# VIDILabs/open-volume-renderer

Hardware: AMD Instinct MI355X
Metric: Msamples/s (primary ray-march samples after ERT); fps alongside (higher is better)
Workload: dtype f32

## Files before the change

### open-volume-renderer_amd/csrc/ovr_hip_kernels.hip

```cpp
#include "ovr_hip_device.h"

namespace ovrhip {
static_assert(kPoolSubs <= 64 && (kPoolSubs & (kPoolSubs - 1)) == 0, "reduce_counters_kernel reduces the sub-pool counters with one wave");
__global__ __launch_bounds__(kBlock) void composite_kernel(const RayMarchParams P)
{
  const int lane = threadIdx.x & 63, wave = threadIdx.x >> 6;
  int ix, iy;
  const bool active = assign_pixel_quad(P, lane, wave, ix, iy) && (lane & 3) == 0;
  const PoolDesc& Q = P.pool;
  if (Q.ctrl[1] != 0u) return;
  const unsigned int tile = blockIdx.x * kWaves + wave;
  const unsigned int pixel_index = (unsigned int)ix + (unsigned int)iy * (unsigned int)P.width;
  float alpha = 0.f;
  unsigned int first = 0;
  int pend = 0;
  if (active) {
    const float4 st = Q.pix_state[pixel_index];
    alpha = st.x; first = __float_as_uint(st.y); pend = __float_as_int(st.z);
  }
  f3 color = mk3(0, 0, 0), gradient = mk3(0, 0, 0);
  const unsigned int total = Q.tile_count[tile];
  auto load_chunk = [&](int c, unsigned int n) {
    ShadeReq r;
    r.px = r.py = r.pz = r.s = r.v = r.tr = r.a = 0.f; r.next = 0;
    if ((unsigned int)lane < n) r = Q.reqs[(size_t)c * 64 + lane];
    return r;
  };
  int c = total > 0u ? Q.tile_first[tile] : 0;
  int link = total > 0u ? Q.chunk_next[c | (kRun - 1)] : 0;
  ShadeReq r = load_chunk(c, min(total, 64u));
  for (unsigned int base = 0; base < total; base += 64u) {
    const unsigned int n = min(total - base, 64u);
    const bool more = base + 64u < total;
    const bool run_end = (c & (kRun - 1)) == kRun - 1;
    const int c_next = run_end ? link : c + 1;
    ShadeReq r_next = r;
    if (more) {
      r_next = load_chunk(c_next, min(total - base - 64u, 64u));
      if (run_end) link = Q.chunk_next[c_next | (kRun - 1)];
    }
    apply_batch(r, base, n, lane, pend, first, color, gradient);
    r = r_next;
    c = c_next;
  }
  if (active) {
    f3 o_c = mk3(0, 0, 0), o_g = mk3(0, 0, 0);
    if (alpha > 0.f) {
      o_c = mk3(color.x / alpha, color.y / alpha, color.z / alpha);
      o_g = mk3(gradient.x / alpha, gradient.y / alpha, gradient.z / alpha);
    }
    float o_a = alpha;
    if (P.spp > 1) {
      float4* sr = reinterpret_cast<float4*>(P.spp_sum_rgba) + pixel_index;
      float* sg = P.spp_sum_grad + 3ull * pixel_index;
      float4 acc = make_float4(0.f, 0.f, 0.f, 0.f);
      f3 accg = mk3(0, 0, 0);
      if (P.spp_index > 0) { acc = *sr; accg = mk3(sg[0], sg[1], sg[2]); }
      acc.x += o_c.x; acc.y += o_c.y; acc.z += o_c.z; acc.w += alpha;
      accg.x += o_g.x; accg.y += o_g.y; accg.z += o_g.z;
      if (P.spp_index + 1 < P.spp) {
        *sr = acc; sg[0] = accg.x; sg[1] = accg.y; sg[2] = accg.z;
        return;
      }
      if (Q.ctrl[32 * (kPoolSubs + 1)] > Q.sub_capacity) return;
      const float rspp = 1.f / (float)P.spp;
      o_a = acc.w * rspp;
      o_c = mk3(acc.x * rspp, acc.y * rspp, acc.z * rspp);
      o_g = mk3(accg.x * rspp, accg.y * rspp, accg.z * rspp);
    }
    write_pixel(P, pixel_index, o_c, o_a, o_g);
  }
}

__global__ __launch_bounds__(256) void reduce_counters_kernel(const unsigned int* __restrict__ partials, int n_blocks, const unsigned int* __restrict__ shade_partials,
                                                             int n_shade_blocks, unsigned long long* counters, unsigned int* pool_ctrl,
                                                             unsigned long long* publish, unsigned int* done, unsigned int* conv_asked)
{
  if (pool_ctrl && blockIdx.x == 0 && threadIdx.x < 64) {
    unsigned int v = threadIdx.x < (unsigned int)kPoolSubs ? pool_ctrl[32u * (threadIdx.x + 1u)] : 0u;
#pragma unroll
    for (int off = 32; off > 0; off >>= 1) v = max(v, (unsigned int)__shfl_xor((int)v, off));
    if (threadIdx.x == 0) atomicMax(&pool_ctrl[32 * (kPoolSubs + 1)], v);
  }
  __shared__ unsigned long long red[4][kNC];
  unsigned long long acc[kNC] = {};
  const int stride = gridDim.x * 256;
  for (int b = blockIdx.x * 256 + threadIdx.x; b < n_blocks; b += stride) {
#pragma unroll
    for (int c = 0; c < kNC; ++c) acc[c] += partials[(size_t)b * kNC + c];
  }
  if (shade_partials)
    for (int b = blockIdx.x * 256 + threadIdx.x; b < n_shade_blocks; b += stride) {
      acc[3] += shade_partials[2 * b];
      acc[6] += shade_partials[2 * b + 1];
    }
#pragma unroll
  for (int c = 0; c < kNC; ++c) {
    for (int off = 32; off > 0; off >>= 1) acc[c] += __shfl_down(acc[c], off);
  }
  const int lane = threadIdx.x & 63, wave = threadIdx.x >> 6;
  if (lane == 0) {
#pragma unroll
    for (int c = 0; c < kNC; ++c) red[wave][c] = acc[c];
  }
  __syncthreads();
  if (threadIdx.x < kNC) atomicAdd(&counters[threadIdx.x], red[0][threadIdx.x] + red[1][threadIdx.x] + red[2][threadIdx.x] + red[3][threadIdx.x]);
  if (!publish) return;
  __shared__ unsigned int ticket;
  __threadfence();
  __syncthreads();
  if (threadIdx.x == 0) ticket = atomicAdd(done, 1u);
  __syncthreads();
  if (ticket != gridDim.x - 1u) return;
  __threadfence();
  if (threadIdx.x < 8) {
    publish[threadIdx.x] = threadIdx.x < kNC ? __hip_atomic_load(&counters[threadIdx.x], __ATOMIC_RELAXED, __HIP_MEMORY_SCOPE_AGENT) : 0ull;
    counters[threadIdx.x] = 0ull;
  }
  unsigned int* pub_ctrl = reinterpret_cast<unsigned int*>(publish + 8);
  if (pool_ctrl)
    for (int i = threadIdx.x; i < kPoolCtrlWords; i += 256) {
      const unsigned int w = __hip_atomic_load(&pool_ctrl[i], __ATOMIC_RELAXED, __HIP_MEMORY_SCOPE_AGENT);
      pub_ctrl[i] = w;
      pool_ctrl[i] = 0u;
      if (conv_asked && i == 32 * (kPoolSubs + 1)) *conv_asked = w;
    }
  else if (conv_asked && threadIdx.x == 0) *conv_asked = 0u;
  if (threadIdx.x == 0) *done = 0u;
}
constexpr int kSchedClasses = 64;
__device__ __forceinline__ float schedule_probe(const RayMarchParams& P, const MarchConsts& mc, unsigned int e, int k)
{
  const f3 c0 = ld3(P.cam_dir), h0 = ld3(P.cam_hor), v0 = ld3(P.cam_ver);
  const f3 oo = to_object(mc, ld3(P.cam_pos));
  const int bx = (int)(e & 0xffffu) * 8, by = (int)(e >> 16) * 8;
  const int ix = min(bx + (k == 0 ? 4 : (k & 1) ? 0 : 7), P.width - 1), iy = min(by + (k == 0 ? 4 : (k & 2) ? 0 : 7), P.height - 1);
  const float ux = ((float)ix + .5f) / (float)P.width - 0.5f, uy = ((float)iy + .5f) / (float)P.height - 0.5f;
  const f3 d = normalize3_exact(mk3(c0.x + ux * h0.x + uy * v0.x, c0.y + ux * h0.y + uy * v0.y, c0.z + ux * h0.z + uy * v0.z));
  float a = 0.f, b = FLT_MAX;
  if (intersect_unit_box(a, b, oo, mk3(d.x * mc.inv_scale.x, d.y * mc.inv_scale.y, d.z * mc.inv_scale.z))) return b - a;
  return -1.f;
}
__device__ __forceinline__ unsigned int schedule_class_of(const RayMarchParams& P, float longest)
{
  if (!(longest >= 0.f)) return 0u;
  const float rel = longest / (P.long_ray_steps * P.step);
  return (unsigned int)min(kSchedClasses - 1, 1 + (int)(rel * (float)(kSchedClasses - 2)));
}

__global__ __launch_bounds__(256) void schedule_classify_kernel(const RayMarchParams P, const unsigned int* __restrict__ src, unsigned int n, int exact,
                                                               unsigned int* __restrict__ cls)
{
  VolConsts vc;
  MarchConsts mc;
  setup_consts(P, vc, mc);
  const unsigned int i = blockIdx.x * 4u + (threadIdx.x >> 6);
  if (i >= n) return;
  const int lane = threadIdx.x & 63;
  const unsigned int e = src[i];
  const int ix = (int)(e & 0xffffu) * 8 + (lane & 7), iy = (int)(e >> 16) * 8 + (lane >> 3);
  bool active = ix < P.width && iy < P.height;
  if (P.world > 1 && active) active = ((ix / P.tile_w + iy / P.tile_h) % P.world) == P.rank;
  const bool hit = exact == 1 && active && pixel_ray_hits_box(P, mc, ix, iy);
  const unsigned long long any = __ballot(hit), act = __ballot(active);
  bool culled = false;
  if (exact == 2) {
    const float x0 = ((float)((int)(e & 0xffffu) * 8) - 1.5f) / (float)P.width - 0.5f, x1 = ((float)((int)(e & 0xffffu) * 8 + 8) + 1.5f) / (float)P.width - 0.5f;
    const float y0 = ((float)((int)(e >> 16) * 8) - 1.5f) / (float)P.height - 0.5f, y1 = ((float)((int)(e >> 16) * 8 + 8) + 1.5f) / (float)P.height - 0.5f;
    const f3 cd = ld3(P.cam_dir), ch = ld3(P.cam_hor), cv = ld3(P.cam_ver);
    auto ray = [&](int k) {
      const float ux = (k == 1 || k == 2) ? x1 : x0, uy = (k >= 2) ? y1 : y0;
      return mk3((cd.x + ux * ch.x + uy * cv.x) * mc.inv_scale.x, (cd.y + ux * ch.y + uy * cv.y) * mc.inv_scale.y, (cd.z + ux * ch.z + uy * cv.z) * mc.inv_scale.z);
    };
    const f3 oo = to_object(mc, ld3(P.cam_pos));
    const int pl = (lane >> 3) & 3, cn = lane & 7;
    const f3 a = ray(pl), b = ray((pl + 1) & 3), in = ray((pl + 2) & 3);
    const f3 nrm = mk3(a.y * b.z - a.z * b.y, a.z * b.x - a.x * b.z, a.x * b.y - a.y * b.x);
    const float side = dot3(nrm, in);
    const f3 v = mk3((float)(cn & 1) - oo.x, (float)((cn >> 1) & 1) - oo.y, (float)(cn >> 2) - oo.z);
    const float d = dot3(nrm, v) * (side >= 0.f ? 1.f : -1.f);
    const float scale = sqrtf(dot3(nrm, nrm) * dot3(v, v));
    const bool outside = lane < 32 && fabsf(side) > 0.f && d < -1e-4f * scale;
    const unsigned int bits = (unsigned int)__ballot(outside);
    bool beyond = false;
#pragma unroll
    for (int k = 0; k < 4; ++k) beyond = beyond || ((bits >> (8 * k)) & 0xffu) == 0xffu;
    bool sign_safe = true;
#pragma unroll
    for (int k = 0; k < 3; ++k) {
      const float c00 = k == 0 ? ray(0).x : k == 1 ? ray(0).y : ray(0).z, c10 = k == 0 ? ray(1).x : k == 1 ? ray(1).y : ray(1).z;
      const float c11 = k == 0 ? ray(2).x : k == 1 ? ray(2).y : ray(2).z, c01 = k == 0 ? ray(3).x : k == 1 ? ray(3).y : ray(3).z;
      const float lo = fminf(fminf(c00, c10), fminf(c11, c01)), hi = fmaxf(fmaxf(c00, c10), fmaxf(c11, c01));
      const float len = sqrtf(dot3(ray(0), ray(0)));
      sign_safe = sign_safe && (lo > 1e-6f * len || hi < -1e-6f * len);
    }
    culled = beyond && sign_safe;
  }
  float longest = lane < 5 ? schedule_probe(P, mc, e, lane) : -1.f;
#pragma unroll
  for (int off = 1; off < 8; off <<= 1) longest = fmaxf(longest, __shfl_xor(longest, off));
  if (lane == 0) {
    unsigned int c = schedule_class_of(P, longest);
    if (exact == 1) c = any != 0ull ? max(c, 1u) : 0u;
    if (exact == 2) c = culled ? 0u : max(c, 1u);
    cls[i] = c | ((unsigned int)__popcll(act) << 8);
  }
}

constexpr int kSchedRow = kSchedClasses + 1;
__global__ __launch_bounds__(1024) void schedule_hist_kernel(const unsigned int* __restrict__ cls, unsigned int n, unsigned int* __restrict__ hist)
{
  __shared__ unsigned int count[kSchedRow];
  if (threadIdx.x < kSchedRow) count[threadIdx.x] = 0u;
  __syncthreads();
  const unsigned int i = blockIdx.x * 1024u + threadIdx.x;
  if (i < n) {
    const unsigned int c = cls[i];
    atomicAdd(&count[c & 0xffu], 1u);
    if ((c & 0xffu) == 0u) atomicAdd(&count[kSchedClasses], c >> 8);
  }
  __syncthreads();
  if (threadIdx.x < kSchedRow) hist[blockIdx.x * kSchedRow + threadIdx.x] = count[threadIdx.x];
}

__global__ __launch_bounds__(1024) void schedule_scatter_kernel(const unsigned int* __restrict__ src, const unsigned int* __restrict__ cls_in, unsigned int n,
                                                                const unsigned int* __restrict__ hist, unsigned int* __restrict__ dst, unsigned int* __restrict__ info)
{
  __shared__ unsigned int base[kSchedRow], total[kSchedRow];
  __shared__ unsigned int wave_count[16][kSchedClasses];
  const int lane = threadIdx.x & 63, wave = threadIdx.x >> 6;
  if (threadIdx.x < kSchedRow) {
    unsigned int before = 0u, all = 0u;
    for (unsigned int w = 0; w < gridDim.x; ++w) {
      const unsigned int h = hist[w * kSchedRow + threadIdx.x];
      before += w < blockIdx.x ? h : 0u;
      all += h;
    }
    base[threadIdx.x] = before;
    total[threadIdx.x] = all;
  }
  for (int k = threadIdx.x; k < 16 * kSchedClasses; k += 1024) (&wave_count[0][0])[k] = 0u;
  __syncthreads();
  if (threadIdx.x == 0) {
    unsigned int at = 0u;
    for (int c = kSchedClasses - 1; c >= 0; --c) { const unsigned int t = total[c]; base[c] += at; at += t; }
    if (info && blockIdx.x == 0) { info[0] = n - total[0]; info[1] = total[kSchedClasses]; }
  }
  const unsigned int i = blockIdx.x * 1024u + threadIdx.x;
  const bool valid = i < n;
  const unsigned int e = valid ? src[i] : 0u;
  const unsigned int cls = valid ? (cls_in[i] & 0xffu) : 0u;
  unsigned int rank = 0u;
  unsigned long long todo = __ballot(valid);
  while (todo != 0ull) {
    const int leader = __builtin_ctzll(todo);
    const unsigned int lc = (unsigned int)__builtin_amdgcn_readlane((int)cls, leader);
    const unsigned long long same = __ballot(valid && cls == lc);
    if (valid && cls == lc) rank = (unsigned int)__popcll(same & ((1ull << lane) - 1ull));
    if (lane == leader) wave_count[wave][lc] = (unsigned int)__popcll(same);
    todo &= ~same;
  }
  __syncthreads();
  if (threadIdx.x < kSchedClasses) {
    unsigned int run = base[threadIdx.x];
    for (int w = 0; w < 16; ++w) { const unsigned int t = wave_count[w][threadIdx.x]; wave_count[w][threadIdx.x] = run; run += t; }
  }
  __syncthreads();
  if (valid) dst[wave_count[wave][cls] + rank] = e;
}

size_t schedule_workspace_elems(unsigned int n) { return (size_t)((n + 1023u) / 1024u) * kSchedRow + (size_t)n; }

hipError_t launch_schedule(const RayMarchParams& p, const unsigned int* src, unsigned int n, unsigned int* dst, unsigned int* workspace, int exact, unsigned int* info,
                           hipStream_t stream)
{
  if (n == 0) {
    return hipSuccess;
  }
  const dim3 grid((n + 1023u) / 1024u);
  unsigned int* hist = workspace;
  unsigned int* cls = workspace + (size_t)grid.x * kSchedRow;
  hipLaunchKernelGGL(schedule_classify_kernel, dim3((n + 3u) / 4u), dim3(256), 0, stream, p, src, n, exact, cls);
  hipLaunchKernelGGL(schedule_hist_kernel, grid, dim3(1024), 0, stream, cls, n, hist);
  hipLaunchKernelGGL(schedule_scatter_kernel, grid, dim3(1024), 0, stream, src, cls, n, hist, dst, info);
  return hipGetLastError();
}

__global__ __launch_bounds__(256) void clear_blocks_kernel(const RayMarchParams P, const unsigned int* __restrict__ blocks, unsigned int n, int clear_accum)
{
  const unsigned int i = blockIdx.x * 4u + (threadIdx.x >> 6);
  if (i >= n) return;
  const int lane = threadIdx.x & 63;
  const unsigned int e = blocks[i];
  const int ix = (int)(e & 0xffffu) * 8 + (lane & 7), iy = (int)(e >> 16) * 8 + (lane >> 3);
  bool active = ix < P.width && iy < P.height;
  if (P.world > 1 && active) active = ((ix / P.tile_w + iy / P.tile_h) % P.world) == P.rank;
  if (!active) return;
  const size_t pi = (size_t)ix + (size_t)iy * (size_t)P.width;
  reinterpret_cast<float4*>(P.rgba)[pi] = make_float4(0.f, 0.f, 0.f, 0.f);
  if (P.grad) { float* g = P.grad + 3 * pi; g[0] = 0.f; g[1] = 0.f; g[2] = 0.f; }
  if (clear_accum && P.accum) reinterpret_cast<float4*>(P.accum)[pi] = make_float4(0.f, 0.f, 0.f, 0.f);
  if (clear_accum && P.accum_half) reinterpret_cast<float4*>(P.accum_half)[pi] = make_float4(0.f, 0.f, 0.f, 0.f);
}
hipError_t launch_clear_blocks(const RayMarchParams& p, const unsigned int* blocks, unsigned int n, int clear_accum, hipStream_t stream)
{
  if (n == 0) return hipSuccess;
  hipLaunchKernelGGL(clear_blocks_kernel, dim3((n + 3u) / 4u), dim3(256), 0, stream, p, blocks, n, clear_accum);
  return hipGetLastError();
}

__device__ __forceinline__ bool convergence_attempt_void(const ConvergenceParams& C) { return C.words[2] > C.sub_capacity; }

__global__ __launch_bounds__(256) void convergence_kernel(const ConvergenceParams C)
{
  const unsigned int i = blockIdx.x * 4u + (threadIdx.x >> 6);
  if (i >= C.n_active) return;
  if (convergence_attempt_void(C)) return;
  const int lane = threadIdx.x & 63;
  const unsigned int ent = C.active[i];
  const int bx = (int)(ent & 0xffffu), by = (int)(ent >> 16);
  const int ix = bx * 8 + (lane & 7), iy = by * 8 + (lane >> 3);
  bool present = ix < C.width && iy < C.height;
  if (C.world > 1 && present) present = ((ix / C.tile_w + iy / C.tile_h) % C.world) == C.rank;
  const size_t pi = (size_t)(present ? ix : 0) + (size_t)(present ? iy : 0) * (size_t)C.width;
  float e = 0.f;
  if (present) {
    const float4 a = reinterpret_cast<const float4*>(C.accum)[pi], h = reinterpret_cast<const float4*>(C.accum_half)[pi];
    const float fn = (float)C.frame_index, fh = (float)(C.frame_index / 2);
    const float mr = a.x / fn, mg = a.y / fn, mb = a.z / fn, ma = a.w / fn;
    const float hr = h.x / fh, hg = h.y / fh, hb = h.z / fh, ha = h.w / fh;
    const float d = ((fabsf(mr - hr) + fabsf(mg - hg)) + fabsf(mb - hb)) + fabsf(ma - ha);
    const float s = ((mr + mg) + mb) + ma;
    e = s > 0.f ? d / sqrtf(s) : 0.f;
  }
  const int count = (int)__popcll(__ballot(present));
#pragma unroll
  for (int off = 1; off < 64; off <<= 1) e += __shfl_xor(e, off);
  const float E = count > 0 ? e / (float)count : 0.f;
  const bool retire = C.adaptive != 0 && E <= C.threshold;
  if (lane == 0) {
    const size_t b = (size_t)bx + (size_t)by * (size_t)C.blocks_x;
    C.block_error[b] = E;
    C.block_frames[b] = retire ? -C.frame_index : C.frame_index;
    unsigned int* w = &C.words[retire ? 1 : 0];
    const unsigned int bits = __float_as_uint(E);
    if (bits > __hip_atomic_load(w, __ATOMIC_RELAXED, __HIP_MEMORY_SCOPE_AGENT)) atomicMax(w, bits);
// ... 1340 lines not shown
```

Baseline: 95230.

## Prefetch request chunks in groups of four and apply per-quad via DPP broadcasts

The composite kernel now walks the tile's shade-request chunks in groups of four matching the reservation sequence, keeping two groups in flight (triple-buffered register groups) so global loads overlap compositing. Each chunk is applied with a new quad-cooperative routine where all four lanes of a pixel quad fetch four consecutive requests via bperm and broadcast them with DPP, replacing the per-request batch application. This aims to hide load latency and cut serialized per-sample shuffles, at the cost of much higher register pressure from holding up to 12 chunks and a more intricate chunk-link traversal.

New measurement: 96020, median of 2. Within noise of the previous version (+0.8%).

```diff
diff --git a/open-volume-renderer_amd/csrc/ovr_hip_kernels.hip b/open-volume-renderer_amd/csrc/ovr_hip_kernels.hip
--- a/open-volume-renderer_amd/csrc/ovr_hip_kernels.hip
+++ b/open-volume-renderer_amd/csrc/ovr_hip_kernels.hip
@@ -2,11 +2,52 @@
 
 namespace ovrhip {
 static_assert(kPoolSubs <= 64 && (kPoolSubs & (kPoolSubs - 1)) == 0, "reduce_counters_kernel reduces the sub-pool counters with one wave");
+template <int B>
+__device__ __forceinline__ int quad_bcast_i(int x) { return __builtin_amdgcn_update_dpp(0, x, B * 0x55, 0xf, 0xf, true); }
+
+__device__ __forceinline__ void apply_chunk_quads(const ShadeReq& res, unsigned int base, unsigned int n, int lane, int& pend, unsigned int& first, f3& color,
+                                                  f3& gradient)
+{
+  const int sub = lane & 3;
+  for (;;) {
+    const bool has = (pend > 0) && ((first - base) < n);
+    if (__ballot(has) == 0ull) break;
+    const int j = has ? (int)((first - base) & ~3u) + sub : lane;
+    const float tcx = bperm(j, res.px), tcy = bperm(j, res.py), tcz = bperm(j, res.pz);
+    const float tgx = bperm(j, res.s), tgy = bperm(j, res.v), tgz = bperm(j, res.tr);
+    const float ta = bperm(j, res.a);
+    const int tn = bperm_i(j, res.next);
+    int applied = 0;
+#define OVR_SLOT(B)                                                                                                            \
+    {                                                                                                                          \
+      const float a = quad_bcast<B>(ta);                                                                                       \
+      const bool on = has && a > 0.f;                                                                                          \
+      const float cx = fmaf(quad_bcast<B>(tcx), a, color.x), cy = fmaf(quad_bcast<B>(tcy), a, color.y);                        \
+      const float cz = fmaf(quad_bcast<B>(tcz), a, color.z);                                                                   \
+      const float gx = fmaf(quad_bcast<B>(tgx), a, gradient.x), gy = fmaf(quad_bcast<B>(tgy), a, gradient.y);                  \
+      const float gz = fmaf(quad_bcast<B>(tgz), a, gradient.z);                                                                \
+      const int nx = quad_bcast_i<B>(tn);                                                                                      \
+      color.x = on ? cx : color.x; color.y = on ? cy : color.y; color.z = on ? cz : color.z;                                   \
+      gradient.x = on ? gx : gradient.x; gradient.y = on ? gy : gradient.y; gradient.z = on ? gz : gradient.z;                 \
+      first = on ? (unsigned int)nx : first;                                                                                   \
+      applied += on ? 1 : 0;                                                                                                   \
+    }
+    OVR_SLOT(0) OVR_SLOT(1) OVR_SLOT(2) OVR_SLOT(3)
+#undef OVR_SLOT
+    if (has) pend = applied > 0 ? pend - applied : 0;
+  }
+}
+
+__device__ __forceinline__ int uniform(int x) { return __builtin_amdgcn_readfirstlane(x); }
+
+struct ChunkGroup { ShadeReq r[kRun]; };
+
 __global__ __launch_bounds__(kBlock) void composite_kernel(const RayMarchParams P)
 {
   const int lane = threadIdx.x & 63, wave = threadIdx.x >> 6;
   int ix, iy;
-  const bool active = assign_pixel_quad(P, lane, wave, ix, iy) && (lane & 3) == 0;
+  const bool in_image = assign_pixel_quad(P, lane, wave, ix, iy);
+  const bool active = in_image && (lane & 3) == 0;
   const PoolDesc& Q = P.pool;
   if (Q.ctrl[1] != 0u) return;
   const unsigned int tile = blockIdx.x * kWaves + wave;
@@ -14,34 +55,69 @@
   float alpha = 0.f;
   unsigned int first = 0;
   int pend = 0;
-  if (active) {
+  if (in_image) {
     const float4 st = Q.pix_state[pixel_index];
     alpha = st.x; first = __float_as_uint(st.y); pend = __float_as_int(st.z);
   }
   f3 color = mk3(0, 0, 0), gradient = mk3(0, 0, 0);
-  const unsigned int total = Q.tile_count[tile];
-  auto load_chunk = [&](int c, unsigned int n) {
-    ShadeReq r;
-    r.px = r.py = r.pz = r.s = r.v = r.tr = r.a = 0.f; r.next = 0;
-    if ((unsigned int)lane < n) r = Q.reqs[(size_t)c * 64 + lane];
-    return r;
+  static_assert(kRun == 4 && kRunMax == 4 * kRun, "the composite's walk follows the reservation sequence 4, 8, 16, 16, ... in groups of 4 chunks");
+  const unsigned int total = (unsigned int)uniform((int)Q.tile_count[tile]);
+  const unsigned int n_chunks = (total + 63u) / 64u, n_groups = (n_chunks + kRun - 1u) / kRun;
+  auto chunk_len = [&](unsigned int g, int i) {
+    const unsigned int at = (g * kRun + (unsigned int)i) * 64u;
+    return at < total ? min(total - at, 64u) : 0u;
   };
-  int c = total > 0u ? Q.tile_first[tile] : 0;
-  int link = total > 0u ? Q.chunk_next[c | (kRun - 1)] : 0;
-  ShadeReq r = load_chunk(c, min(total, 64u));
-  for (unsigned int base = 0; base < total; base += 64u) {
-    const unsigned int n = min(total - base, 64u);
-    const bool more = base + 64u < total;
-    const bool run_end = (c & (kRun - 1)) == kRun - 1;
-    const int c_next = run_end ? link : c + 1;
-    ShadeReq r_next = r;
-    if (more) {
-      r_next = load_chunk(c_next, min(total - base - 64u, 64u));
-      if (run_end) link = Q.chunk_next[c_next | (kRun - 1)];
-    }
-    apply_batch(r, base, n, lane, pend, first, color, gradient);
-    r = r_next;
-    c = c_next;
+  auto apply_group = [&](const ChunkGroup& G, unsigned int g) {
+#pragma unroll
+    for (int i = 0; i < kRun; ++i) apply_chunk_quads(G.r[i], (g * kRun + (unsigned int)i) * 64u, chunk_len(g, i), lane, pend, first, color, gradient);
+  };
+  if (n_groups == 1u) {
+    const int cb = uniform(Q.tile_first[tile]);
+    ChunkGroup G;
+#pragma unroll
+    for (int i = 0; i < kRun; ++i) {
+      ShadeReq r;
+      r.px = r.py = r.pz = r.s = r.v = r.tr = r.a = 0.f; r.next = 0;
+      if ((unsigned int)lane < chunk_len(0u, i)) r = Q.reqs[(size_t)(cb + i) * 64 + lane];
+      G.r[i] = r;
+    }
+    apply_group(G, 0u);
+  }
+  else if (n_groups > 1u) {
+    auto load_group = [&](int cb, unsigned int g) {
+      const int valid = g < n_groups ? (int)min(n_chunks - g * kRun, (unsigned int)kRun) : 1;
+      ChunkGroup G;
+#pragma unroll
+      for (int i = 0; i < kRun; ++i) G.r[i] = Q.reqs[(size_t)(cb + min(i, valid - 1)) * 64 + lane];
+      return G;
+    };
+    auto last_of_reservation = [](unsigned int g) { return g == 0u || (g & 3u) == 2u; };
+    int cb = uniform(Q.tile_first[tile]);
+    int link = Q.chunk_next[cb + kRun - 1];
+    ChunkGroup G0 = load_group(cb, 0u);
+    cb = uniform(link);
+    if (n_groups > 3u) link = Q.chunk_next[cb + 2 * kRun - 1];
+    ChunkGroup G1 = load_group(cb, 1u), G2;
+    auto step = [&](const ChunkGroup& cur, ChunkGroup& ahead, unsigned int g) {
+      if (g + 2u < n_groups) {
+        if (last_of_reservation(g + 1u)) {
+          cb = uniform(link);
+          if (g + 6u < n_groups) link = Q.chunk_next[cb + kRunMax - 1];
+        }
+        else cb += kRun;
+      }
+      else if (g + 2u == n_groups) cb += (int)(n_chunks - 1u - (g + 1u) * kRun);
+      ahead = load_group(cb, g + 2u);
+      apply_group(cur, g);
+    };
+    for (unsigned int g = 0;; g += 3u) {
+      step(G0, G2, g);
+      if (g + 1u >= n_groups) break;
+      step(G1, G0, g + 1u);
+      if (g + 2u >= n_groups) break;
+      step(G2, G1, g + 2u);
+      if (g + 3u >= n_groups) break;
+    }
   }
   if (active) {
     f3 o_c = mk3(0, 0, 0), o_g = mk3(0, 0, 0);
```
